# Anton-Le/PhysicsBasedBayesianInference

Measured on AMD Instinct MI355X. Metric: leapfrog-steps*chains/sec (node); d=128 Gaussian, ensemble=65536, higher is better.
Workload: dtype f64; 1 GPU; C2: d=128 dense-precision Gaussian, fp64, L=10 leapfrog steps per HMC iteration, in-kernel Philox momentum + Metropolis; chains_per_gpu=65536, total_chains=65536, D=128, L=10, parallelism=ensemble-sharded x1, draw=f32 (single-precision Box-Muller on the transcendental unit; momenta only)

## Files before the change

### physicsbasedbayesianinference_amd/csrc/kernels_dense.hip

```cpp
#include "kernels_dense_dev.h"

namespace {

struct DenseEvalPrm {
    const double* frag;
    const double* mu;
    const double* q;
    const double* p;
    const double* mass;
    double* U_out;
    double* grad_out;
    double* w_out;
    int64_t N, ldn;
    double cst;
    int D, mode;
};

template <int NT, bool FULL>
__global__ void __launch_bounds__(BLOCK, 1) k_dense_eval(DenseEvalPrm prm) {
    constexpr int DP = 16 * NT;
    constexpr int KS = 4 * NT;
    extern __shared__ __attribute__((aligned(16))) char smem[];
    v2f64* frag2 = reinterpret_cast<v2f64*>(smem);
    double* mu = reinterpret_cast<double*>(smem + (size_t)DP * DP * sizeof(double));
// ... 188 lines not shown
        return pbbi_fail(PBBI_ERR_UNSUPPORTED,
                         "dense kernels address a lane's rows with 32-bit offsets: padded D * "
                         "leading stride must be < 2^29 elements; shard the ensemble");
    return PBBI_OK;
}

int check(const pbbi_potential* pot) {
    if (pot->dtype != PBBI_F64)
        return pbbi_fail(PBBI_ERR_UNSUPPORTED, "dense Gaussian kernels are fp64 only in this build");
    if (pot->DP == 0 || pot->d_frag == nullptr)
        return pbbi_fail(PBBI_ERR_UNSUPPORTED,
                         "dense Gaussian: register-resident MFMA path needs D <= 128 (D = " +
                             std::to_string(pot->D) + ")");
    return PBBI_OK;
}

}

int dense_build_fragments(pbbi_potential* pot, const double* P, const double* mean) {
    const int D = pot->D;
    pot->DP = 0;
    pot->d_frag = nullptr;
    pot->d_mean_pad = nullptr;
    if (D > 128 || pot->dtype != PBBI_F64) return PBBI_OK;
    const int DP = D <= 32 ? 32 : (D <= 64 ? 64 : (D <= 96 ? 96 : 128));
    const int NT = DP / 16, KS = DP / 4;
    std::vector<double> frag((size_t)DP * DP, 0.0), mu((size_t)DP, 0.0);
    for (int s = 0; s < KS; ++s)
        for (int t = 0; t < NT; ++t)
            for (int l = 0; l < 64; ++l) {
                const int i = 16 * t + (l & 15), k = 4 * s + (l >> 4);
                const double val = (i < D && k < D) ? P[(size_t)i * D + k] : 0.0;
                frag[(((size_t)s * (NT / 2) + t / 2) * 64 + l) * 2 + (t & 1)] = val;
            }
    pot->zero_mean = true;
    for (int d = 0; d < D; ++d) {
        mu[d] = mean ? mean[d] : 0.0;
        if (mu[d] != 0.0) pot->zero_mean = false;
    }
    PBBI_HIP(hipMalloc(&pot->d_frag, frag.size() * sizeof(double)));
    PBBI_HIP(hipMalloc(&pot->d_mean_pad, mu.size() * sizeof(double)));
    PBBI_HIP(hipMemcpy(pot->d_frag, frag.data(), frag.size() * sizeof(double), hipMemcpyHostToDevice));
    PBBI_HIP(hipMemcpy(pot->d_mean_pad, mu.data(), mu.size() * sizeof(double), hipMemcpyHostToDevice));
    pot->DP = DP;
    return PBBI_OK;
}

int dense_hmc_iter(const IterArgs& a) {
    if (int rc = check(a.pot)) return rc;
    if (pbbi_dyn(a) && (a.method != PBBI_LEAPFROG || a.L < 1))
        return pbbi_fail(PBBI_ERR_UNSUPPORTED, "per-chain trajectory lengths on the dense kernel: Leapfrog with L >= 1");
    if (int rc = check_ld(a.pot, a.ldn_in > a.ldn_out ? a.ldn_in : a.ldn_out)) return rc;
    if (a.N == 0) return PBBI_OK;
    DensePrm prm{};
#ifdef PBBI_STAMPS
    prm.stamps = g_stamp_buf;
#endif
    prm.frag = (const double*)a.pot->d_frag;
    prm.mu = (const double*)a.pot->d_mean_pad;
    prm.q_in = (const double*)a.q_in;
    prm.p_in = (const double*)a.p_in;
    prm.u_in = (const double*)a.u_in;
    prm.mass = (const double*)a.mass;
    prm.q_out = (double*)a.q_out;
    prm.p_out = (double*)a.p_out;
    prm.v_out = nullptr;
    prm.ratio_out = (double*)a.ratio_out;
    prm.reject_out = a.reject_out;
    prm.N = a.N; prm.ldn_in = a.ldn_in; prm.ldn_out = a.ldn_out;
    prm.h = a.h; prm.cst = a.pot->cst; prm.kT = a.kT;
    prm.L = a.L; prm.D = a.pot->D; prm.flags = a.flags; prm.rng = a.rng; prm.mode = 0;
    prm.seed = a.seed; prm.iter = a.iter; prm.chain0 = a.chain0;
    prm.steps_in = a.steps_in; prm.steps_out = a.steps_out;
    int carry = 0;
    if (a.carry && a.carry_g && a.carry_sel && dense_carry_applies(a)) {
        carry = a.carry;
        prm.carry_g = (double*)a.carry_g;
        prm.carry_sel = a.carry_sel;
        prm.carry_slab_bytes = (uint32_t)((uint64_t)a.pot->DP * (uint64_t)a.N * 8u);
    }
    if (a.fuse_S > 1) {
        if (carry == 0 || a.ldn_in != a.ldn_out || !a.rng)
            return pbbi_fail(PBBI_ERR_INVALID, "fused dense iterations belong to a carried run (internal)");
        prm.fuse_first = (carry == 1);
        carry = 2;
        prm.fuse_S = a.fuse_S;
        prm.fuse_wrap2 = a.fuse_wrap2;
        prm.fuse_slab0 = a.fuse_slab0;
        prm.fuse_slab = (int64_t)a.pot->D * a.N;
        prm.fuse_q_base = (double*)a.fuse_q_base;
    } else if (carry != 0 && a.method == PBBI_STORMER_VERLET) {
        if (!a.rng) return pbbi_fail(PBBI_ERR_INVALID, "carried dense iterations draw in the kernel (internal)");
        prm.fuse_first = (carry == 1);
        carry = 2;
        prm.fuse_S = 1;
        prm.fuse_wrap2 = 0;
        prm.fuse_slab0 = 0;
        prm.fuse_slab = (int64_t)a.pot->D * a.N;
        prm.fuse_q_base = (double*)a.q_out;
    }
    return launch_traj(a.pot, a.method, prm, a.N, a.stream, carry);
}

int dense_fused_iterations(const IterArgs& a) {
    static const int chunk = [] {
        const char* e = getenv("PBBI_DENSE_FUSE");
// ... 66 lines not shown
```

### physicsbasedbayesianinference_amd/csrc/pbbi_api.hip

```cpp
#include <dlfcn.h>

#include <cmath>
#include <cstring>
#include <new>
#include <vector>

#include <type_traits>

#include "pbbi_internal.h"
#include "pbbi_chain.h"
#include "pbbi_rng.h"

static thread_local std::string g_last_error;

void pbbi_set_error(const std::string& msg) { g_last_error = msg; }
int pbbi_fail(int code, const std::string& msg) {
    g_last_error = msg;
    return code;
}

int pbbi_num_cus(int device) {
    static int cached[64] = {0};
    if (device >= 0 && device < 64 && cached[device]) return cached[device];
    int cus = 0;
// ... 584 lines not shown
int pbbi_device_count(int* count_out) {
    if (!count_out) return pbbi_fail(PBBI_ERR_INVALID, "count_out is NULL");
    *count_out = 0;
    PBBI_HIP(hipGetDeviceCount(count_out));
    return PBBI_OK;
}

int pbbi_device_info(int device, pbbi_devinfo* out) {
    if (!out) return pbbi_fail(PBBI_ERR_INVALID, "out is NULL");
    hipDeviceProp_t prop;
    PBBI_HIP(hipGetDeviceProperties(&prop, device));
    std::memset(out, 0, sizeof(*out));
    std::strncpy(out->name, prop.name, sizeof(out->name) - 1);
    std::strncpy(out->arch, prop.gcnArchName, sizeof(out->arch) - 1);
    out->compute_units = prop.multiProcessorCount;
    out->hbm_bytes = (int64_t)prop.totalGlobalMem;
    out->lds_bytes_per_block = (int)prop.sharedMemPerBlock;
    out->clock_khz = prop.clockRate;
    return PBBI_OK;
}

int pbbi_potential_create_harmonic(int D, const double* springConsts, int dtype, int device,
                                   pbbi_potential** out) {
    if (!springConsts) return pbbi_fail(PBBI_ERR_INVALID, "springConsts is NULL");
    if (int rc = new_handle(KIND_HARMONIC, D, dtype, device, out)) return rc;
    DeviceGuard guard(device);
    int rc = upload_padded(springConsts, D, dtype, &(*out)->d_prec);
    if (rc == PBBI_OK) rc = upload_mean(*out, nullptr);
    return finish_or_destroy(rc, out);
}

int pbbi_potential_create_gauss_diag(int D, const double* mean, const double* prec, double cst,
                                     int dtype, int device, pbbi_potential** out) {
    if (!prec) return pbbi_fail(PBBI_ERR_INVALID, "prec is NULL");
    if (int rc = new_handle(KIND_GAUSS_DIAG, D, dtype, device, out)) return rc;
    DeviceGuard guard(device);
    (*out)->cst = cst;
    int rc = upload_padded(prec, D, dtype, &(*out)->d_prec);
    if (rc == PBBI_OK) rc = upload_mean(*out, mean);
    return finish_or_destroy(rc, out);
}

int pbbi_potential_create_gauss_dense(int D, const double* mean, const double* precision,
                                      double cst, int dtype, int device, pbbi_potential** out) {
    if (!precision) return pbbi_fail(PBBI_ERR_INVALID, "precision is NULL");
    if (int rc = new_handle(KIND_GAUSS_DENSE, D, dtype, device, out)) return rc;
    DeviceGuard guard(device);
    (*out)->cst = cst;
    int rc = upload(precision, (size_t)D * D, dtype, &(*out)->d_prec);
    if (rc == PBBI_OK) rc = upload_mean(*out, mean);
    if (rc == PBBI_OK) rc = dense_build_fragments(*out, precision, mean);
    if (rc == PBBI_OK && (*out)->DP == 0) rc = big_build(*out, precision, mean);
    if (rc == PBBI_OK && (*out)->DP == 0) rc = dense_stream_build(*out, precision, mean);
    return finish_or_destroy(rc, out);
}

int pbbi_potential_create_rosenbrock(int D, double a, double b, double s, int dtype, int device,
                                     pbbi_potential** out) {
    if (!(s != 0.0)) return pbbi_fail(PBBI_ERR_INVALID, "Rosenbrock scale s must be non-zero");
    if (int rc = new_handle(KIND_ROSENBROCK, D, dtype, device, out)) return rc;
    (*out)->a = a; (*out)->b = b; (*out)->s = s;
    return PBBI_OK;
}

int pbbi_potential_create_custom(const char* plugin_path, int D, const double* params, int n_params,
                                 int dtype, int device, pbbi_potential** out) {
    if (!plugin_path) return pbbi_fail(PBBI_ERR_INVALID, "plugin_path is NULL");
    if (n_params < 0 || (n_params > 0 && !params))
        return pbbi_fail(PBBI_ERR_INVALID, "params is NULL / n_params < 0");
    if (int rc = new_handle(KIND_CUSTOM, D, dtype, device, out)) return rc;
    pbbi_potential* p = *out;
    DeviceGuard guard(device);
    p->plugin = dlopen(plugin_path, RTLD_NOW | RTLD_LOCAL);
    if (!p->plugin) {
        const char* why = dlerror();
        return finish_or_destroy(pbbi_fail(PBBI_ERR_INVALID, std::string("cannot load the potential plugin: ") +
                                                                 (why ? why : plugin_path)), out);
    }
    auto abi = (int (*)(void))dlsym(p->plugin, "pbbi_plugin_abi");
    auto pdt = (int (*)(void))dlsym(p->plugin, "pbbi_plugin_dtype");
    p->plugin_hmc_iter = (int (*)(const IterArgs*))dlsym(p->plugin, "pbbi_plugin_hmc_iter");
    p->plugin_integrate = (int (*)(const IntegrateArgs*))dlsym(p->plugin, "pbbi_plugin_integrate");
    p->plugin_eval = (int (*)(const EvalArgs*, int))dlsym(p->plugin, "pbbi_plugin_eval");
    int rc = PBBI_OK;
    if (!abi || !pdt || !p->plugin_hmc_iter || !p->plugin_integrate || !p->plugin_eval)
        rc = pbbi_fail(PBBI_ERR_INVALID, "plugin does not export the pbbi_plugin_* entry points");
    else if (abi() != PBBI_PLUGIN_ABI)
        rc = pbbi_fail(PBBI_ERR_INVALID, "plugin was built against another libpbbi (ABI " +
                                             std::to_string(abi()) + ", expected " +
                                             std::to_string(PBBI_PLUGIN_ABI) + "): rebuild it");
    else if (pdt() != dtype)
        rc = pbbi_fail(PBBI_ERR_INVALID, "plugin was built for the other dtype");
    if (rc == PBBI_OK) {
        p->n_params = n_params;
        rc = upload(params, (size_t)n_params, dtype, &p->d_params);
    }
    return finish_or_destroy(rc, out);
}

int pbbi_potential_create_glm(int D, int64_t M, const double* X, const double* y, int family,
                              double prior_precision, int dtype, int device, pbbi_potential** out) {
    if (!X || !y) return pbbi_fail(PBBI_ERR_INVALID, "X / y is NULL");
    if (M < 1) return pbbi_fail(PBBI_ERR_INVALID, "M must be >= 1");
    if (family != PBBI_GLM_LOGISTIC && family != PBBI_GLM_POISSON)
        return pbbi_fail(PBBI_ERR_INVALID, "unknown GLM family");
    if (!(prior_precision >= 0.0)) return pbbi_fail(PBBI_ERR_INVALID, "prior_precision must be >= 0");
    if (out) *out = nullptr;
    if (D > 128 || dtype == PBBI_F32)
        return pbbi_fail(PBBI_ERR_UNSUPPORTED, "GLM potentials run on the fp64 matrix-core kernels: float64 and "
                                               "D <= 128 only");
    if (int rc = new_handle(KIND_GLM, D, dtype, device, out)) return rc;
    DeviceGuard guard(device);
    return finish_or_destroy(glm_build(*out, M, X, y, family, prior_precision), out);
}

int pbbi_glm_pack_design(int D, int64_t M, const double* X, double* out, int64_t out_len, int64_t* len_out) {
    if (D < 1 || D > 128 || M < 1) return pbbi_fail(PBBI_ERR_INVALID, "need 1 <= D <= 128 and M >= 1");
    const int64_t len = glm_image_len(D, M);
    if (len_out) *len_out = len;
    if (!out) return PBBI_OK;
    if (!X) return pbbi_fail(PBBI_ERR_INVALID, "X is NULL");
    if (out_len < len) return pbbi_fail(PBBI_ERR_INVALID, "out is shorter than the image");
    glm_pack(D, M, X, out);
    return PBBI_OK;
}

int pbbi_potential_destroy(pbbi_potential* pot) {
    if (!pot) return PBBI_OK;
    DeviceGuard guard(pot->device);
    for (void* p : {pot->d_mean, pot->d_prec, pot->d_frag, pot->d_mean_pad, pot->d_big_PT, pot->d_big_mu,
                    pot->d_sfrag, pot->d_smean, pot->d_params, pot->d_glm_img, pot->d_glm_y})
        if (p) (void)hipFree(p);
    if (pot->plugin) (void)dlclose(pot->plugin);
    delete pot;
    return PBBI_OK;
}

int pbbi_potential_dim(const pbbi_potential* pot) { return pot ? pot->D : PBBI_ERR_INVALID; }
int pbbi_potential_dtype(const pbbi_potential* pot) { return pot ? pot->dtype : PBBI_ERR_INVALID; }
int pbbi_potential_device(const pbbi_potential* pot) { return pot ? pot->device : PBBI_ERR_INVALID; }

int pbbi_potential_eval(const pbbi_potential* pot, const void* q, int64_t N, int64_t ldn,
                        void* U_out, void* grad_out, void* stream) {
    if (int rc = check_common(pot, N, ldn)) return rc;
    if (!q && N > 0) return pbbi_fail(PBBI_ERR_INVALID, "q is NULL");
    DeviceGuard guard(pot->device);
    EvalArgs a{pot, q, nullptr, nullptr, N, ldn, U_out, grad_out, nullptr, 0, (hipStream_t)stream};
    return route_eval(a);
}

int pbbi_integrate(const pbbi_potential* pot, int method, void* q, void* p, const void* mass,
                   void* v_out, int64_t N, int64_t ldn, double h, int L, void* stream) {
    if (int rc = check_common(pot, N, ldn)) return rc;
    if (method != PBBI_LEAPFROG && method != PBBI_STORMER_VERLET)
        return pbbi_fail(PBBI_ERR_INVALID, "Invalid integration method selected.");
    if (L < 0) return pbbi_fail(PBBI_ERR_INVALID, "numSteps must be >= 0");
    if ((!q || !p) && N > 0) return pbbi_fail(PBBI_ERR_INVALID, "q / p is NULL");
    DeviceGuard guard(pot->device);
    IntegrateArgs a{pot, method, q, p, mass, v_out, N, ldn, h, L, (hipStream_t)stream};
    return route_integrate(a);
}

int pbbi_leapfrog(const pbbi_potential* pot, void* q, void* p, const void* mass, int64_t N,
                  int64_t ldn, double h, int L, void* stream) {
    return pbbi_integrate(pot, PBBI_LEAPFROG, q, p, mass, nullptr, N, ldn, h, L, stream);
}

int pbbi_stormer_verlet(const pbbi_potential* pot, void* q, void* p, const void* mass, int64_t N,
                        int64_t ldn, double h, int L, void* stream) {
    return pbbi_integrate(pot, PBBI_STORMER_VERLET, q, p, mass, nullptr, N, ldn, h, L, stream);
}

int pbbi_energy(const pbbi_potential* pot, const void* q, const void* p, const void* mass,
                int64_t N, int64_t ldn, void* H_out, void* weight_out, void* stream) {
    if (int rc = check_common(pot, N, ldn)) return rc;
    if ((!q || !p) && N > 0) return pbbi_fail(PBBI_ERR_INVALID, "q / p is NULL");
    DeviceGuard guard(pot->device);
    EvalArgs a{pot, q, p, mass, N, ldn, H_out, nullptr, weight_out, 0, (hipStream_t)stream};
    return route_energy(a);
}

int pbbi_weights_ratio(const pbbi_potential* pot, const void* newQ, const void* newP,
                       const void* oldQ, const void* oldP, const void* mass, int64_t N,
                       int64_t ldn, void* ratio_out, void* stream) {
    if (int rc = check_common(pot, N, ldn)) return rc;
    if (!ratio_out && N > 0) return pbbi_fail(PBBI_ERR_INVALID, "ratio_out is NULL");
// ... 241 lines not shown
    if (N == 0 || R < 2 || parity + 1 >= R) return PBBI_OK;
    if (!q || !betas) return pbbi_fail(PBBI_ERR_INVALID, "q / betas is NULL");
    DeviceGuard guard(pot->device);
    hipStream_t st = (hipStream_t)stream;
    Scratch ws(st);
    void* U = ws.get((size_t)N * elem_size(pot->dtype));
    if (!U) return pbbi_fail(PBBI_ERR_HIP, "hipMallocAsync failed for the potential energies");
    EvalArgs e{pot, q, nullptr, nullptr, N, ldn, U, nullptr, nullptr, 0, st};
    if (int rc = route_eval(e)) return rc;
    const int pairs = (R - parity) / 2;
    const dim3 grid((unsigned)((Nr + 255) / 256), (unsigned)pairs), block(256);
    if (pot->dtype == PBBI_F64)
        hipLaunchKernelGGL(k_replica_exchange<double>, grid, block, 0, st, (double*)q, ldn, (const double*)U, betas,
                           pot->D, Nr, R, parity, seed, iter, chain0, swapped_out);
    else
        hipLaunchKernelGGL(k_replica_exchange<float>, grid, block, 0, st, (float*)q, ldn, (const float*)U, betas,
                           pot->D, Nr, R, parity, seed, iter, chain0, swapped_out);
    PBBI_HIP(hipGetLastError());
    return PBBI_OK;
}

int pbbi_describe_run(const pbbi_potential* pot, int method, int64_t N, int64_t ldn, int L, int S, int flags,
                      char* out, int out_len) {
    if (int rc = hmc_check(pot, method, N, ldn, L)) return rc;
    if (!out || out_len < 1) return pbbi_fail(PBBI_ERR_INVALID, "out buffer missing");
    IterArgs a{};
    a.pot = pot; a.method = method; a.N = N; a.ldn_in = ldn; a.ldn_out = N; a.L = L; a.flags = flags; a.rng = 1;
    a.kT = 1.0;
    a.carry = 2; a.carry_g = (void*)(uintptr_t)16; a.carry_sel = (uint8_t*)(uintptr_t)16;
    std::string d;
    int fuse = 1;
    if (pot->kind == KIND_GLM) {
        d = "k_glm: GLM likelihood as two fp64 MFMA products per gradient (eta = X W, g = X^T r), 16 chains per wave, X "
            "staged through LDS in blocks of 16 observations (rows padded to " + std::to_string(pot->glm_DP) + ")";
        fuse = 1;
    } else if (pot->kind == KIND_CUSTOM) {
        d = "user-potential plugin kernels (one chain per lane; registers up to D = 16 / 32, workspace beyond)";
        fuse = route_fused_iterations(a);
    } else if (is_big(pot) && dense_stream_applies(a)) {
        d = "k_dense_hmc (streamed P): register-resident MFMA kernel, 16 chains per wave, one wave per SIMD, the "
            "precision matrix streamed through an LDS ring (rows padded to " + std::to_string(pot->DPS) + ")";
        const bool carry = S >= 2 && dense_stream_carry_applies(a);
        d += carry ? "; gradient carried between iterations: yes (L mat-vecs per iteration)"
                   : "; gradient carried between iterations: no (L + 1 mat-vecs per iteration)";
        if (!carry) a.carry = 0;
        fuse = carry ? dense_stream_fused_iterations(a) : 1;
    } else if (is_big(pot)) {
        d = "kernels_big: one fused MFMA GEMM per leapfrog step over the whole ensemble";
        d += big_carry_applies(a) && S >= 2 ? "; gradient carried between iterations: yes (L GEMMs per iteration)"
                                            : "; gradient carried between iterations: no (L + 1 GEMMs per iteration)";
    } else if (is_dense(pot)) {
        d = "k_dense_hmc: register-resident MFMA kernel, 16 chains per wave";
        const bool carry = S >= 2 && dense_carry_applies(a);
        if (carry) {
            d += "; gradient carried between iterations: yes (L mat-vecs per iteration)";
        } else {
            d += "; gradient carried between iterations: no (L + 1 mat-vecs per iteration) -- ";
            const uint64_t lim = (PBBI_CARRY_MAX_BYTES - 1) / ((uint64_t)pot->DP * 16u);
            if (S < 2) d += "a run of one iteration";
            else if (L < 1 || pbbi_dyn(a)) d += "runs of a fixed trajectory length L >= 1 only";
            else if ((uint64_t)N > lim)
                d += "the two carried-gradient slabs (D*N*16 bytes) must stay below 2^32 for 32-bit buffer offsets: "
                     "at D = " + std::to_string(pot->D) + " (rows padded to " + std::to_string(pot->DP) + ") that is N <= " + std::to_string(lim) +
                     " chains per call; shard the ensemble or split the call";
            else d += "switched off (PBBI_NO_CARRY / PBBI_DENSE_V1)";
        }
        if (!carry) a.carry = 0;
        fuse = carry ? dense_fused_iterations(a) : 1;
    } else {
        d = lane_route_name(a);
        fuse = lane_fused_iterations(a);
    }
    d += "; iterations per launch: up to " + std::to_string(fuse < 1 ? 1 : fuse);
    if (flags & PBBI_DRAW_F64) d += "; momentum draw: double precision";
    snprintf(out, (size_t)out_len, "%s", d.c_str());
    return PBBI_OK;
}

int pbbi_philox_normal(uint64_t seed, int rng_stream, uint64_t iter, uint64_t chain0, int D,
                       int64_t N, int64_t ldn, double scale, const void* scale_per_chain,
                       int dtype, int device, void* out, void* stream) {
    if (D < 1 || N < 0 || ldn < N) return pbbi_fail(PBBI_ERR_INVALID, "bad D / N / ldn");
    if (iter > UINT32_MAX) return pbbi_fail(PBBI_ERR_INVALID, "iter must be < 2^32");
    if (!out && N > 0) return pbbi_fail(PBBI_ERR_INVALID, "out is NULL");
    if (N == 0) return PBBI_OK;
    DeviceGuard guard(device);
    const dim3 grid((unsigned)((N + 255) / 256)), block(256);
    if (dtype == PBBI_F64)
        hipLaunchKernelGGL(k_philox_normal<double>, grid, block, 0, (hipStream_t)stream, seed,
                           rng_stream, iter, chain0, D, N, ldn, scale,
                           (const double*)scale_per_chain, (double*)out);
    else if (dtype == PBBI_F32)
        hipLaunchKernelGGL(k_philox_normal<float>, grid, block, 0, (hipStream_t)stream, seed,
                           rng_stream, iter, chain0, D, N, ldn, scale, (const float*)scale_per_chain,
                           (float*)out);
    else
        return pbbi_fail(PBBI_ERR_INVALID, "unknown dtype");
    PBBI_HIP(hipGetLastError());
    return PBBI_OK;
}

int pbbi_philox_steps(uint64_t seed, uint64_t iter, uint64_t chain0, int64_t N, int L, int device,
                      int32_t* out, void* stream) {
    if (N < 0 || L < 0) return pbbi_fail(PBBI_ERR_INVALID, "bad N / L");
    if (iter > UINT32_MAX) return pbbi_fail(PBBI_ERR_INVALID, "iter must be < 2^32");
    if (!out && N > 0) return pbbi_fail(PBBI_ERR_INVALID, "out is NULL");
    if (N == 0) return PBBI_OK;
// ... 174 lines not shown
```

### physicsbasedbayesianinference_amd/csrc/pbbi_internal.h

```cpp
#pragma once
#include <hip/hip_runtime.h>
#include <stdint.h>

#include <string>

#include "pbbi.h"

enum { KIND_HARMONIC = 0, KIND_GAUSS_DIAG = 1, KIND_GAUSS_DENSE = 2, KIND_ROSENBROCK = 3, KIND_CUSTOM = 4, KIND_GLM = 5 };

#define PBBI_PLUGIN_ABI 4

struct IterArgs;
struct IntegrateArgs;
struct EvalArgs;

struct pbbi_potential {
    int kind;
    int D;
    int dtype;
    int device;
    double cst, a, b, s;
    void* d_mean;
    void* d_prec;
    int DP;
    void* d_frag;
    void* d_mean_pad;
    bool zero_mean;
    int DPAD_big;
    void* d_big_PT;
    void* d_big_mu;
    void* plugin;
    void* d_params;
    int n_params;
    int (*plugin_hmc_iter)(const IterArgs*);
    int (*plugin_integrate)(const IntegrateArgs*);
    int (*plugin_eval)(const EvalArgs*, int mode);
    int DPS;
    void* d_sfrag;
    void* d_smean;
    int glm_DP;
    int glm_family;
    int64_t glm_M;
    double glm_lam;
    void* d_glm_img;
    void* d_glm_y;
};

void pbbi_set_error(const std::string& msg);
int pbbi_fail(int code, const std::string& msg);

#define PBBI_HIP(expr)                                                                          \
    do {                                                                                        \
        hipError_t _e = (expr);                                                                 \
        if (_e != hipSuccess)                                                                   \
            return pbbi_fail(PBBI_ERR_HIP, std::string(#expr) + ": " + hipGetErrorString(_e)); \
    } while (0)

struct DeviceGuard {
    int prev = -1;
    bool ok = true;
    explicit DeviceGuard(int dev) {
        if (hipGetDevice(&prev) != hipSuccess) { ok = false; return; }
        if (prev != dev && hipSetDevice(dev) != hipSuccess) ok = false;
    }
    ~DeviceGuard() {
        if (prev >= 0) (void)hipSetDevice(prev);
    }
};

__host__ __device__ inline double pbbi_accept_beta(int flags, double kT) {
    return (flags & PBBI_BETA_ACCEPT) ? 1.0 / kT : 1.0;
}

int pbbi_num_cus(int device);
struct IterArgs {
    const pbbi_potential* pot;
    int method;
    const void* q_in;
    const void* p_in;
    const void* u_in;
    const void* mass;
    void* q_out;
    void* p_out;
    void* ratio_out;
    uint8_t* reject_out;
    int64_t N, ldn_in, ldn_out;
    double h;
    int L;
    int flags;
    int rng;
    uint64_t seed, iter, chain0;
    double kT;
    hipStream_t stream;
    void* scratch;
    size_t scratch_bytes;
    size_t* scratch_used;
    int fuse_S;
    int fuse_wrap2;
// ... 56 lines not shown
        void* p = nullptr;
        if (hipMallocAsync(&p, bytes, st) != hipSuccess) return nullptr;
        owned.push_back(p);
        return p;
    }
    ~Scratch() {
        for (void* p : owned) (void)hipFreeAsync(p, st);
        if (used) *used = total;
    }
};

int lane_hmc_iter(const IterArgs& a);
int lane_integrate(const IntegrateArgs& a);
int lane_eval(const EvalArgs& a);
int lane_energy(const EvalArgs& a);
bool lane2_applies(const IterArgs& a);
int lane2_hmc_iter(const IterArgs& a);
int lane_fused_iterations(const IterArgs& a);
const char* lane_route_name(const IterArgs& a);
int lane_dyn_hmc_iter(const IterArgs& a);
bool lane_gist_applies(const pbbi_potential* pot);
int lane_gist_iter(const IterArgs& a);
bool sepn_applies(const IterArgs& a);
int sepn_hmc_iter(const IterArgs& a);
bool sepx_applies(const IterArgs& a);
int sepx_hmc_iter(const IterArgs& a);
bool rosn_applies(const IterArgs& a);
int rosn_hmc_iter(const IterArgs& a);
bool rosg_applies(const IterArgs& a);
int rosg_hmc_iter(const IterArgs& a);
bool rosgx_applies(const IterArgs& a);
int rosgx_hmc_iter(const IterArgs& a);
int stream_hmc_iter(const IterArgs& a);
int stream_integrate(const IntegrateArgs& a);
int stream_eval(const EvalArgs& a);
int stream_energy(const EvalArgs& a);
#define PBBI_CARRY_MAX_BYTES (((uint64_t)1 << 32) - ((uint64_t)1 << 20))
int dense_hmc_iter(const IterArgs& a);
bool dense_carry_applies(const IterArgs& a);
int dense_fused_iterations(const IterArgs& a);
bool big_carry_applies(const IterArgs& a);
void big_carry_bytes(const pbbi_potential* pot, int64_t N, size_t* g_bytes, size_t* sel_bytes);
int dense_integrate(const IntegrateArgs& a);
int dense_eval(const EvalArgs& a);
int dense_energy(const EvalArgs& a);
int dense_build_fragments(pbbi_potential* pot, const double* precision_host, const double* mean_host);
int dense_stream_build(pbbi_potential* pot, const double* precision_host, const double* mean_host);
bool dense_stream_applies(const IterArgs& a);
bool dense_stream_carry_applies(const IterArgs& a);
int dense_stream_fused_iterations(const IterArgs& a);
int dense_stream_hmc_iter(const IterArgs& a);
bool dense_stream_integrate_applies(const IntegrateArgs& a);
int dense_stream_integrate(const IntegrateArgs& a);
int big_hmc_iter(const IterArgs& a);
int big_integrate(const IntegrateArgs& a);
int big_eval(const EvalArgs& a);
int big_energy(const EvalArgs& a);
int big_build(pbbi_potential* pot, const double* precision_host, const double* mean_host);
int glm_build(pbbi_potential* pot, int64_t M, const double* X, const double* y, int family, double lam);
int glm_padded_dim(int D);
int64_t glm_image_len(int D, int64_t M);
void glm_pack(int D, int64_t M, const double* X, double* out);
int glm_hmc_iter(const IterArgs& a);
int glm_integrate(const IntegrateArgs& a);
int glm_eval(const EvalArgs& a);
int glm_energy(const EvalArgs& a);
```

Before: 2.086 billion leapfrog-steps*chains/s.

## Apply L leapfrog steps as one precomputed linear propagator for dense Gaussians

For a D=128 fp64 dense Gaussian, leapfrog dynamics are linear, so the L steps collapse into one map. The map's blocks are built from a host-side Jacobi eigendecomposition of the precision matrix and baked into device images, cached per (h, L). A new MFMA kernel then does a fixed five mat-vecs per HMC iteration instead of L, streaming the images through an LDS ring with buffer-to-LDS loads. The cost is setup work, extra device memory for the images and eigenvectors, and rounding that can differ from stepwise integration. The path runs only when L is at least 7 and no per-chain mass is given.

```diff
diff --git a/physicsbasedbayesianinference_amd/csrc/kernels_dense.hip b/physicsbasedbayesianinference_amd/csrc/kernels_dense.hip
--- a/physicsbasedbayesianinference_amd/csrc/kernels_dense.hip
+++ b/physicsbasedbayesianinference_amd/csrc/kernels_dense.hip
@@ -264,6 +264,7 @@
         return pbbi_fail(PBBI_ERR_UNSUPPORTED, "per-chain trajectory lengths on the dense kernel: Leapfrog with L >= 1");
     if (int rc = check_ld(a.pot, a.ldn_in > a.ldn_out ? a.ldn_in : a.ldn_out)) return rc;
     if (a.N == 0) return PBBI_OK;
+    if (a.carry && a.carry_g && a.carry_sel && dense_prop_applies(a)) return dense_prop_hmc_iter(a);
     DensePrm prm{};
 #ifdef PBBI_STAMPS
     prm.stamps = g_stamp_buf;
diff --git a/physicsbasedbayesianinference_amd/csrc/kernels_dprop.hip b/physicsbasedbayesianinference_amd/csrc/kernels_dprop.hip
--- /dev/null
+++ b/physicsbasedbayesianinference_amd/csrc/kernels_dprop.hip
@@ -0,0 +1,557 @@
+#include <cmath>
+#include <mutex>
+
+#include "kernels_dense_dev.h"
+
+namespace {
+
+constexpr int PROP_MIN_L_DEFAULT = 7;
+
+struct PropCfg {
+    static constexpr int CHUNK = 16384;
+    static constexpr int RING = 4;
+    static constexpr int DMA = 4;
+    static constexpr int NCYC = 40;
+    static constexpr int C_A1 = 0, C_G = 8, C_B = 16, C_A2 = 24, C_P = 32;
+    static constexpr int LDS_RING = RING * CHUNK;
+    static constexpr int LDS = LDS_RING + 128 * 8;
+    static constexpr size_t IMG_DOUBLES = (size_t)NCYC * CHUNK / 8;
+};
+
+__device__ __forceinline__ void pr_issue_part(const PRing& r, int ci, int m) {
+    using C = PropCfg;
+    typedef __attribute__((address_space(3))) void lds_void;
+    const int slot = ci % C::RING;
+    __builtin_amdgcn_raw_ptr_buffer_load_lds(r.src, (lds_void*)(r.lds + slot * C::CHUNK + m * 4096), 16, r.voff,
+                                             (uint32_t)(ci * C::CHUNK + m * 4096) + r.woff, 0, 0);
+}
+
+template <int KC, bool INLOOP>
+__device__ __forceinline__ void pr_acquire() {
+    using C = PropCfg;
+    constexpr int YOUNGER = INLOOP ? C::DMA * (C::RING - 3) + (C::DMA < KC - 1 ? C::DMA : KC - 1) : C::DMA * (C::RING - 2);
+    asm volatile("s_waitcnt vmcnt(%0) lgkmcnt(0)\n\ts_barrier" ::"n"(YOUNGER) : "memory");
+}
+
+template <int HP, int C0, bool ZERO, typename XF, typename PF>
+__device__ __forceinline__ void prop_pass(const PRing& r, const v2f64* __restrict__ ringL, v4f64 (&acc)[2 * HP], XF xat,
+                                          PF pre) {
+    using C = PropCfg;
+    constexpr int KS = 32, KC = 16 / HP, H1 = (HP + 1) / 2;
+    auto frag_at = [&](int s, int t2) -> v2f64 {
+        const int slot = (C0 + s / KC) % C::RING;
+        return ringL[((slot * KC + s % KC) * HP + t2) * 64];
+    };
+    pr_acquire<KC, false>();
+    v2f64 A[HP], An[HP];
+#pragma unroll
+    for (int t2 = 0; t2 < HP; ++t2) A[t2] = frag_at(0, t2);
+    if constexpr (ZERO) {
+#pragma unroll
+        for (int t = 0; t < 2 * HP; ++t) acc[t] = v4f64{0.0, 0.0, 0.0, 0.0};
+    }
+    double x = xat(0);
+#pragma unroll
+    for (int s = 0; s < KS; ++s) {
+#pragma unroll
+        for (int t2 = 0; t2 < H1; ++t2) {
+            acc[2 * t2] = __builtin_amdgcn_mfma_f64_16x16x4f64(A[t2].x, x, acc[2 * t2], 0, 0, 0);
+            acc[2 * t2 + 1] = __builtin_amdgcn_mfma_f64_16x16x4f64(A[t2].y, x, acc[2 * t2 + 1], 0, 0, 0);
+        }
+        __builtin_amdgcn_sched_barrier(0);
+        if (s + 1 < KS) {
+            if ((s + 1) % KC == 0) pr_acquire<KC, true>();
+#pragma unroll
+            for (int t2 = 0; t2 < HP; ++t2) An[t2] = frag_at(s + 1, t2);
+            pre(s + 1);
+        }
+        __builtin_amdgcn_sched_barrier(0);
+#pragma unroll
+        for (int t2 = H1; t2 < HP; ++t2) {
+            acc[2 * t2] = __builtin_amdgcn_mfma_f64_16x16x4f64(A[t2].x, x, acc[2 * t2], 0, 0, 0);
+            acc[2 * t2 + 1] = __builtin_amdgcn_mfma_f64_16x16x4f64(A[t2].y, x, acc[2 * t2 + 1], 0, 0, 0);
+        }
+        __builtin_amdgcn_sched_barrier(0);
+        if (s % KC < C::DMA) pr_issue_part(r, (C0 + s / KC + C::RING - 1) % C::NCYC, s % KC);
+        if (s + 1 < KS) x = xat(s + 1);
+#pragma unroll
+        for (int t2 = 0; t2 < HP; ++t2) A[t2] = An[t2];
+    }
+}
+
+__device__ __forceinline__ double dot16(const double* x, const v4f64 (&acc)[4]) {
+    double sum = 0.0;
+#pragma unroll
+    for (int t = 0; t < 4; ++t)
+#pragma unroll
+        for (int r = 0; r < 4; ++r) sum = fma(x[4 * t + r], acc[t][r], sum);
+    return sum;
+}
+
+template <bool ZMEAN, int DRAW>
+__global__ void __launch_bounds__(BLOCK, 2) k_dense_hmc_prop(DensePrm prm) {
+    using C = PropCfg;
+    constexpr int KS = 32;
+    extern __shared__ __attribute__((aligned(16))) char smem[];
+    const int lane = threadIdx.x & 63;
+    const int wave = __builtin_amdgcn_readfirstlane(threadIdx.x >> 6);
+    double* mu = reinterpret_cast<double*>(smem + C::LDS_RING);
+    PRing ring{};
+    ring.src = buf_make(prm.frag);
+    ring.lds = smem + wave * 1024;
+    ring.voff = 16u * (uint32_t)lane;
+    ring.woff = 1024u * (uint32_t)wave;
+    if (prm.fuse_first) {
+#pragma unroll
+        for (int ci = 0; ci < C::RING - 1; ++ci)
+#pragma unroll
+            for (int m = 0; m < C::DMA; ++m) pr_issue_part(ring, C::C_P + ci, m);
+    } else {
+#pragma unroll
+        for (int ci = 0; ci < C::RING - 1; ++ci)
+#pragma unroll
+            for (int m = 0; m < C::DMA; ++m) pr_issue_part(ring, ci, m);
+    }
+    for (int i = threadIdx.x; i < 128; i += BLOCK) mu[i] = prm.mu[i];
+    __syncthreads();
+    if (blockIdx.x & 1) __builtin_amdgcn_s_setprio(1);
+    const int g = lane >> 4;
+    const int c = lane & 15;
+    const v2f64* ringL = reinterpret_cast<const v2f64*>(smem) + lane;
+    const double* muG = mu + g;
+
+    int64_t n0 = ((int64_t)blockIdx.x * 4 + wave) * CHAINS_PER_WAVE;
+    bool ghost = false;
+    if (n0 >= prm.N) {
+        ghost = true;
+        n0 = (prm.N - 1) / CHAINS_PER_WAVE * CHAINS_PER_WAVE;
+    }
+    const int64_t left = prm.N - n0;
+    const bool valid = !ghost && c < left;
+    const int cc = c < left ? c : (int)left - 1;
+    const uint32_t ld_in = 8u * (uint32_t)prm.ldn_in, ld_out = 8u * (uint32_t)prm.ldn_out;
+    const uint32_t vin = (uint32_t)g * ld_in + 8u * (uint32_t)cc, s4in = 4u * ld_in;
+    const uint32_t vout = (uint32_t)g * ld_out + 8u * (uint32_t)cc, s4out = 4u * ld_out;
+    const __amdgpu_buffer_rsrc_t qin = buf_make(prm.q_in + n0);
+    const uint32_t ld_g = 8u * (uint32_t)prm.N, s4g = 4u * ld_g;
+    const uint32_t vg0 = (uint32_t)g * ld_g + 8u * (uint32_t)cc;
+    const __amdgpu_buffer_rsrc_t gbuf = buf_make(prm.carry_g + n0);
+    uint32_t csel = prm.fuse_first ? 0u : prm.carry_sel[n0 + cc];
+    const uint64_t chain = prm.chain0 + (uint64_t)(n0 + cc);
+    const double pstd = sqrt(prm.kT);
+    auto nopre = [](int) {};
+    using I0 = std::integral_constant<int, 0>;
+    using I1 = std::integral_constant<int, 1>;
+
+    double xL[KS];
+    v4f64 acc[8];
+    double xg_cur = 0.0;
+    auto grad_pass = [&](auto pass_c, uint32_t voff) -> double {
+        constexpr int PASS = decltype(pass_c)::value;
+        v4f64 (&a4)[4] = reinterpret_cast<v4f64 (&)[4]>(acc[0]);
+        prop_pass<2, C::C_P + 4 * PASS, true>(ring, ringL, a4, [&](int s) { return xL[s]; }, nopre);
+        if (valid) {
+#pragma unroll
+            for (int t = 0; t < 4; ++t)
+#pragma unroll
+                for (int r = 0; r < 4; ++r) store_row(gbuf, voff, s4g, 4 * (PASS * 4 + t) + r, a4[t][r]);
+        }
+        return dot16(xL + 16 * PASS, a4);
+    };
+    if (prm.fuse_first) {
+#pragma unroll
+        for (int s = 0; s < KS; ++s) {
+            const double qv = load_row(qin, vin, s4in, s);
+            xL[s] = ZMEAN ? qv : qv - muG[4 * s];
+        }
+        xg_cur = grad_pass(I0{}, vg0);
+        xg_cur += grad_pass(I1{}, vg0);
+    } else {
+        const uint32_t vgc = vg0 + (csel ? prm.carry_slab_bytes : 0u);
+        double part[2];
+#pragma unroll
+        for (int pass = 0; pass < 2; ++pass) {
+            double sum = 0.0;
+#pragma unroll
+            for (int i = 0; i < 16; ++i) {
+                const int s = 16 * pass + i;
+                const double qv = load_row(qin, vin, s4in, s);
+                sum = fma(ZMEAN ? qv : qv - muG[4 * s], load_row(gbuf, vgc, s4g, s), sum);
+            }
+            part[pass] = sum;
+        }
+        xg_cur = part[0] + part[1];
+    }
+    __builtin_amdgcn_sched_barrier(0);
+
+#pragma nounroll
+    for (int kf = 0; kf < prm.fuse_S; ++kf) {
+        const uint64_t iter_k = prm.iter + (uint64_t)kf;
+        double* const ratio_k = prm.ratio_out ? prm.ratio_out + (int64_t)kf * prm.N : nullptr;
+        uint8_t* const reject_k = prm.reject_out ? prm.reject_out + (int64_t)kf * prm.N : nullptr;
+        const int64_t s_out = prm.fuse_wrap2 ? ((prm.fuse_slab0 + kf) & 1) : prm.fuse_slab0 + kf;
+        const int64_t s_prev = prm.fuse_wrap2 ? ((prm.fuse_slab0 + kf - 1) & 1) : prm.fuse_slab0 + kf - 1;
+        const __amdgpu_buffer_rsrc_t qin_k = kf > 0 ? buf_make(prm.fuse_q_base + s_prev * prm.fuse_slab + n0) : qin;
+        const uint32_t vq = kf > 0 ? vout : vin, s4q = kf > 0 ? s4out : s4in;
+        const __amdgpu_buffer_rsrc_t qout_k = buf_make(prm.fuse_q_base + s_out * prm.fuse_slab + n0);
+        const __amdgpu_buffer_rsrc_t pout_k = buf_make(prm.p_out + (prm.p_out ? (int64_t)kf * prm.fuse_slab : 0) + n0);
+        const bool have_p = (prm.p_out != nullptr);
+        const uint32_t vg_cur = vg0 + (csel ? prm.carry_slab_bytes : 0u);
+        const uint32_t vg_new = vg0 + (csel ? 0u : prm.carry_slab_bytes);
+
+        double xa[8], xb[8];
+        auto g0_load = [&](double (&dst)[8], int grp) {
+#pragma unroll
+            for (int i = 0; i < 8; ++i) dst[i] = load_row(gbuf, vg_cur, s4g, 8 * grp + i);
+        };
+        auto x0_load = [&](double (&dst)[8], int grp) {
+#pragma unroll
+            for (int i = 0; i < 8; ++i) {
+                const double qv = load_row(qin_k, vq, s4q, 8 * grp + i);
+                dst[i] = qv;
+            }
+        };
+        g0_load(xa, 0);
+
+        double p[KS];
+        const bool draw64 = DRAW == 1;
+#pragma unroll
+        for (int k = 0; k < KS / 4; ++k) {
+            double z[4];
+            rng_normal4d(prm.seed, PBBI_STREAM_MOMENTUM, iter_k, chain, (uint32_t)((k << 2) | g), draw64, z);
+#pragma unroll
+            for (int sl = 0; sl < 4; ++sl) p[4 * k + sl] = z[sl] * pstd;
+            __builtin_amdgcn_sched_barrier(0);
+        }
+        double pp = 0.0;
+#pragma unroll
+        for (int s = 0; s < KS; ++s) pp += p[s] * p[s];
+        const double oldH = 0.5 * chain_sum(pp) + (0.5 * chain_sum(xg_cur) + prm.cst);
+
+        prop_pass<4, C::C_A1, true>(ring, ringL, acc, [&](int s) { return p[s]; }, nopre);
+        prop_pass<4, C::C_G, false>(
+            ring, ringL, acc, [&](int s) { return ((s >> 3) & 1) ? xb[s & 7] : xa[s & 7]; },
+            [&](int s) {
+                if (s % 8 == 1 && s / 8 + 1 < 4) {
+                    if ((s / 8 + 1) & 1) g0_load(xb, s / 8 + 1);
+                    else g0_load(xa, s / 8 + 1);
+                }
+            });
+        __builtin_amdgcn_sched_barrier(0);
+        x0_load(xa, 0);
+        pp = 0.0;
+#pragma unroll
+        for (int t = 0; t < 8; ++t)
+#pragma unroll
+            for (int r = 0; r < 4; ++r) pp += acc[t][r] * acc[t][r];
+        if (have_p && valid) {
+#pragma unroll
+            for (int t = 0; t < 8; ++t)
+#pragma unroll
+                for (int r = 0; r < 4; ++r) store_row(pout_k, vout, s4out, 4 * t + r, acc[t][r]);
+        }
+        __builtin_amdgcn_sched_barrier(0);
+
+        prop_pass<4, C::C_B, true>(ring, ringL, acc, [&](int s) { return p[s]; }, nopre);
+        prop_pass<4, C::C_A2, false>(
+            ring, ringL, acc,
+            [&](int s) {
+                const double qv = ((s >> 3) & 1) ? xb[s & 7] : xa[s & 7];
+                return ZMEAN ? qv : qv - muG[4 * s];
+            },
+            [&](int s) {
+                if (s % 8 == 1 && s / 8 + 1 < 4) {
+                    if ((s / 8 + 1) & 1) x0_load(xb, s / 8 + 1);
+                    else x0_load(xa, s / 8 + 1);
+                }
+            });
+        __builtin_amdgcn_sched_barrier(0);
+#pragma unroll
+        for (int t = 0; t < 8; ++t)
+#pragma unroll
+            for (int r = 0; r < 4; ++r) {
+                const int s = 4 * t + r;
+                const double qv = ZMEAN ? acc[t][r] : acc[t][r] + muG[4 * s];
+                if (valid) store_row(qout_k, vout, s4out, s, qv);
+                xL[s] = ZMEAN ? qv : qv - muG[4 * s];
+            }
+        __builtin_amdgcn_sched_barrier(0);
+
+        double xg_new = grad_pass(I0{}, vg_new);
+        xg_new += grad_pass(I1{}, vg_new);
+
+        const double newH = 0.5 * chain_sum(pp) + (0.5 * chain_sum(xg_new) + prm.cst);
+        const double ratio = exp((oldH - newH) * pbbi_accept_beta(prm.flags, prm.kT));
+        const double u = rng_uniform(prm.seed, iter_k, chain);
+        const bool reject = (ratio == ratio) && (u > (ratio < 1.0 ? ratio : 1.0));
+        if (reject) {
+            const bool compat = (prm.flags & PBBI_COMPAT_P_FROM_OLDQ) != 0;
+#pragma unroll
+            for (int s = 0; s < KS; ++s) xL[s] = load_row(qin_k, vq, s4q, s);
+            if (valid) {
+#pragma unroll
+                for (int s = 0; s < KS; ++s) store_row(qout_k, vout, s4out, s, xL[s]);
+                if (have_p) {
+#pragma unroll
+                    for (int s = 0; s < KS; ++s) store_row(pout_k, vout, s4out, s, compat ? xL[s] : p[s]);
+                }
+            }
+        }
+        csel ^= reject ? 0u : 1u;
+        xg_cur = reject ? xg_cur : xg_new;
+        if (valid && g == 0) {
+            if (ratio_k) ratio_k[n0 + c] = ratio;
+            if (reject_k) reject_k[n0 + c] = reject ? 1 : 0;
+        }
+    }
+    if (valid && g == 0) prm.carry_sel[n0 + c] = (uint8_t)csel;
+    asm volatile("s_waitcnt vmcnt(0)" ::: "memory");
+}
+
+__host__ __device__ inline double prop_vfv(const double* __restrict__ V, const double* __restrict__ f, int i, int k) {
+    double s = 0.0, e = 0.0;
+    for (int m = 0; m < 128; ++m) {
+        const double a = V[i * 128 + m], b = V[k * 128 + m], w = f[m];
+        const double ab = a * b, abe = fma(a, b, -ab);
+        const double t = ab * w, te = fma(ab, w, -t);
+        const double sn = s + t, bb = sn - s;
+        e += ((s - (sn - bb)) + (t - bb)) + (te + abe * w);
+        s = sn;
+    }
+    return s + e;
+}
+
+__global__ void k_prop_images(const double* __restrict__ V, const double* __restrict__ coef ,
+                              const double* __restrict__ P, double* __restrict__ out) {
+    const int idx = blockIdx.x * blockDim.x + threadIdx.x;
+    if (idx >= (int)PropCfg::IMG_DOUBLES) return;
+    const int img = idx / 16384, w = idx % 16384;
+    const int e = w & 1, l = (w >> 1) & 63;
+    int i, k;
+    if (img < 4) {
+        const int t2 = (w >> 7) & 3, s = w >> 9;
+        i = 16 * (2 * t2 + e) + (l & 15);
+        k = 4 * s + (l >> 4);
+    } else {
+        const int t2 = (w >> 7) & 1, s = (w >> 8) & 31, pass = w >> 13;
+        i = 16 * (pass * 4 + 2 * t2 + e) + (l & 15);
+        k = 4 * s + (l >> 4);
+    }
+    const int sel = img == 0 ? 0 : img == 1 ? 1 : img == 2 ? 2 : 0;
+    out[idx] = img == 4 ? P[i * 128 + k] : prop_vfv(V, coef + 128 * sel, i, k);
+}
+
+void jacobi_eig(int n, std::vector<long double>& a, std::vector<long double>& v, std::vector<long double>& w) {
+    v.assign((size_t)n * n, 0.0L);
+    for (int i = 0; i < n; ++i) v[(size_t)i * n + i] = 1.0L;
+    long double norm = 0.0L;
+    for (long double x : a) norm += x * x;
+    for (int sweep = 0; sweep < 60; ++sweep) {
+        long double off = 0.0L;
+        for (int p = 0; p < n; ++p)
+            for (int q = p + 1; q < n; ++q) off += a[(size_t)p * n + q] * a[(size_t)p * n + q];
+        if (off <= 1e-42L * norm) break;
+        for (int p = 0; p < n; ++p)
+            for (int q = p + 1; q < n; ++q) {
+                const long double apq = a[(size_t)p * n + q];
+                if (apq == 0.0L) continue;
+                const long double theta = (a[(size_t)q * n + q] - a[(size_t)p * n + p]) / (2.0L * apq);
+                const long double t = (theta >= 0 ? 1.0L : -1.0L) / (fabsl(theta) + sqrtl(theta * theta + 1.0L));
+                const long double cs = 1.0L / sqrtl(t * t + 1.0L), sn = t * cs;
+                for (int k = 0; k < n; ++k) {
+                    const long double akp = a[(size_t)k * n + p], akq = a[(size_t)k * n + q];
+                    a[(size_t)k * n + p] = cs * akp - sn * akq;
+                    a[(size_t)k * n + q] = sn * akp + cs * akq;
+                }
+                for (int k = 0; k < n; ++k) {
+                    const long double apk = a[(size_t)p * n + k], aqk = a[(size_t)q * n + k];
+                    a[(size_t)p * n + k] = cs * apk - sn * aqk;
+                    a[(size_t)q * n + k] = sn * apk + cs * aqk;
+                }
+                for (int k = 0; k < n; ++k) {
+                    const long double vkp = v[(size_t)k * n + p], vkq = v[(size_t)k * n + q];
+                    v[(size_t)k * n + p] = cs * vkp - sn * vkq;
+                    v[(size_t)k * n + q] = sn * vkp + cs * vkq;
+                }
+            }
+    }
+    w.resize(n);
+    for (int i = 0; i < n; ++i) w[i] = a[(size_t)i * n + i];
+}
+
+void prop_coefficients(const std::vector<long double>& lam, double h, int L, double* a_out, double* g_out, double* b_out) {
+    const long double hl = (long double)h;
+    for (size_t i = 0; i < lam.size(); ++i) {
+        long double a = 1.0L, b = 0.0L, cg = 0.0L, d = 1.0L;
+        const long double l = lam[i];
+        for (int j = 0; j < L; ++j) {
+            cg -= 0.5L * hl * a;  d -= 0.5L * hl * l * b;
+            a += hl * l * cg;     b += hl * d;
+            cg -= 0.5L * hl * a;  d -= 0.5L * hl * l * b;
+        }
+        a_out[i] = (double)(0.5L * (a + d));
+        g_out[i] = (double)cg;
+        b_out[i] = (double)b;
+    }
+}
+
+struct PropCache {
+    std::mutex mtx;
+    std::vector<double> P;
+    std::vector<long double> lam;
+    std::vector<double> V;
+    double* d_V = nullptr;
+    double* d_coef = nullptr;
+    double* d_img = nullptr;
+    double h = 0.0;
+    int L = -1;
+};
+
+void prop_factor(PropCache* pc) {
+    if (!pc->V.empty()) return;
+    std::vector<long double> a(pc->P.begin(), pc->P.end()), v;
+    for (int i = 0; i < 128; ++i)
+        for (int k = i + 1; k < 128; ++k) a[i * 128 + k] = a[k * 128 + i] = 0.5L * (a[i * 128 + k] + a[k * 128 + i]);
+    jacobi_eig(128, a, v, pc->lam);
+    pc->V.assign(v.begin(), v.end());
+}
+
+int prop_images(const pbbi_potential* pot, double h, int L, hipStream_t st, const double** out) {
+    PropCache* pc = (PropCache*)pot->prop;
+    std::lock_guard<std::mutex> lock(pc->mtx);
+    if (pc->d_img && pc->h == h && pc->L == L) {
+        *out = pc->d_img;
+        return PBBI_OK;
+    }
+    prop_factor(pc);
+    if (!pc->d_V) {
+        double* dv = nullptr;
+        PBBI_HIP(hipMalloc((void**)&dv, 128 * 128 * sizeof(double)));
+        if (hipMemcpy(dv, pc->V.data(), 128 * 128 * sizeof(double), hipMemcpyHostToDevice) != hipSuccess) {
+            (void)hipFree(dv);
+            return pbbi_fail(PBBI_ERR_HIP, "propagator set-up: upload of the eigenvectors failed");
+        }
+        pc->d_V = dv;
+    }
+    if (!pc->d_coef) PBBI_HIP(hipMalloc((void**)&pc->d_coef, 3 * 128 * sizeof(double)));
+    if (pc->d_img) (void)hipFree(pc->d_img);
+    pc->d_img = nullptr;
+    pc->L = -1;
+    double coef[3 * 128];
+    prop_coefficients(pc->lam, h, L, coef, coef + 128, coef + 256);
+    PBBI_HIP(hipMemcpy(pc->d_coef, coef, sizeof(coef), hipMemcpyHostToDevice));
+    PBBI_HIP(hipMalloc((void**)&pc->d_img, PropCfg::IMG_DOUBLES * sizeof(double)));
+    hipLaunchKernelGGL(k_prop_images, dim3((unsigned)(PropCfg::IMG_DOUBLES / 256)), dim3(256), 0, st, pc->d_V, pc->d_coef,
+                       (const double*)pot->d_prec, pc->d_img);
+    PBBI_HIP(hipGetLastError());
+    pc->h = h;
+    pc->L = L;
+    *out = pc->d_img;
+    return PBBI_OK;
+}
+
+}
+
+int dense_prop_build(pbbi_potential* pot, const double* P) {
+    pot->prop = nullptr;
+    if (pot->D != 128 || pot->dtype != PBBI_F64) return PBBI_OK;
+    PropCache* pc = new (std::nothrow) PropCache();
+    if (!pc) return pbbi_fail(PBBI_ERR_INVALID, "out of host memory");
+    pc->P.assign(P, P + 128 * 128);
+    pot->prop = pc;
+    return PBBI_OK;
+}
+
+void dense_prop_destroy(pbbi_potential* pot) {
+    PropCache* pc = (PropCache*)pot->prop;
+    if (!pc) return;
+    for (void* p : {(void*)pc->d_V, (void*)pc->d_coef, (void*)pc->d_img})
+        if (p) (void)hipFree(p);
+    delete pc;
+    pot->prop = nullptr;
+}
+
+bool dense_prop_applies(const IterArgs& a) {
+    static const bool off = (getenv("PBBI_NO_PROPAGATOR") != nullptr);
+    static const int min_l = [] {
+        const char* e = getenv("PBBI_PROP_MIN_L");
+        const int v = e ? atoi(e) : PROP_MIN_L_DEFAULT;
+        return v < 1 ? 1 : v;
+    }();
+    const pbbi_potential* pot = a.pot;
+    return !off && pot->kind == KIND_GAUSS_DENSE && pot->prop != nullptr && pot->DP == 128 && pot->D == 128 &&
+           a.method == PBBI_LEAPFROG && a.mass == nullptr && a.rng && a.L >= min_l && dense_carry_applies(a);
+}
+
+int dense_prop_hmc_iter(const IterArgs& a) {
+    const pbbi_potential* pot = a.pot;
+    if (!dense_prop_applies(a) || !a.carry || !a.carry_g || !a.carry_sel)
+        return pbbi_fail(PBBI_ERR_INVALID, "dense propagator kernel: not applicable (internal)");
+    if ((int64_t)pot->DP * (a.ldn_in > a.ldn_out ? a.ldn_in : a.ldn_out) >= ((int64_t)1 << 29))
+        return pbbi_fail(PBBI_ERR_UNSUPPORTED, "dense kernels address a lane's rows with 32-bit offsets: padded D * "
+                                               "leading stride must be < 2^29 elements; shard the ensemble");
+    if (a.N == 0) return PBBI_OK;
+    const double* img = nullptr;
+    if (int rc = prop_images(pot, a.h, a.L, a.stream, &img)) return rc;
+    DensePrm prm{};
+    prm.frag = img;
+    prm.mu = (const double*)pot->d_mean_pad;
+    prm.q_in = (const double*)a.q_in;
+    prm.q_out = (double*)a.q_out;
+    prm.p_out = (double*)a.p_out;
+    prm.ratio_out = (double*)a.ratio_out;
+    prm.reject_out = a.reject_out;
+    prm.N = a.N; prm.ldn_in = a.ldn_in; prm.ldn_out = a.ldn_out;
+    prm.h = a.h; prm.cst = pot->cst; prm.kT = a.kT;
+    prm.L = a.L; prm.D = pot->D; prm.flags = a.flags; prm.rng = 1; prm.mode = 0;
+    prm.seed = a.seed; prm.iter = a.iter; prm.chain0 = a.chain0;
+    prm.carry_g = (double*)a.carry_g;
+    prm.carry_sel = a.carry_sel;
+    prm.carry_slab_bytes = (uint32_t)((uint64_t)pot->DP * (uint64_t)a.N * 8u);
+    prm.fuse_first = (a.carry == 1);
+    prm.fuse_slab = (int64_t)pot->D * a.N;
+    if (a.fuse_S > 1) {
+        prm.fuse_S = a.fuse_S;
+        prm.fuse_wrap2 = a.fuse_wrap2;
+        prm.fuse_slab0 = a.fuse_slab0;
+        prm.fuse_q_base = (double*)a.fuse_q_base;
+    } else {
+        prm.fuse_S = 1;
+        prm.fuse_wrap2 = 0;
+        prm.fuse_slab0 = 0;
+        prm.fuse_q_base = (double*)a.q_out;
+    }
+    const dim3 grid((unsigned)((a.N + CHAINS_PER_WG - 1) / CHAINS_PER_WG)), block(BLOCK);
+    const size_t lds = PropCfg::LDS;
+#define LAUNCH_P(Z_, DR_)                                                                                  \
+    {                                                                                                      \
+        auto k = k_dense_hmc_prop<Z_, DR_>;                                                                \
+        PBBI_HIP(hipFuncSetAttribute(reinterpret_cast<const void*>(k), hipFuncAttributeMaxDynamicSharedMemorySize, \
+                                     (int)lds));                                                           \
+        hipLaunchKernelGGL(k, grid, block, lds, a.stream, prm);                                            \
+    }
+    const bool d64 = (a.flags & PBBI_DRAW_F64) != 0;
+    if (pot->zero_mean) {
+        if (d64) LAUNCH_P(true, 1) else LAUNCH_P(true, 0)
+    } else {
+        if (d64) LAUNCH_P(false, 1) else LAUNCH_P(false, 0)
+    }
+#undef LAUNCH_P
+    PBBI_HIP(hipGetLastError());
+    return PBBI_OK;
+}
+
+extern "C" int pbbi_debug_propagator_images(int D, const double* P, double h, int L, double* coef_out, double* A_out,
+                                            double* G_out, double* B_out) {
+    if (D != 128 || !P || L < 1 || !coef_out || !A_out || !G_out || !B_out)
+        return pbbi_fail(PBBI_ERR_INVALID, "propagator images: D = 128, L >= 1, non-NULL outputs");
+    PropCache pc;
+    pc.P.assign(P, P + 128 * 128);
+    prop_factor(&pc);
+    prop_coefficients(pc.lam, h, L, coef_out, coef_out + 128, coef_out + 256);
+    double* outs[3] = {A_out, G_out, B_out};
+    for (int im = 0; im < 3; ++im)
+        for (int i = 0; i < 128; ++i)
+            for (int k = 0; k < 128; ++k) outs[im][i * 128 + k] = prop_vfv(pc.V.data(), coef_out + 128 * im, i, k);
+    return PBBI_OK;
+}
diff --git a/physicsbasedbayesianinference_amd/csrc/pbbi_api.hip b/physicsbasedbayesianinference_amd/csrc/pbbi_api.hip
--- a/physicsbasedbayesianinference_amd/csrc/pbbi_api.hip
+++ b/physicsbasedbayesianinference_amd/csrc/pbbi_api.hip
@@ -660,6 +660,7 @@
     if (rc == PBBI_OK) rc = dense_build_fragments(*out, precision, mean);
     if (rc == PBBI_OK && (*out)->DP == 0) rc = big_build(*out, precision, mean);
     if (rc == PBBI_OK && (*out)->DP == 0) rc = dense_stream_build(*out, precision, mean);
+    if (rc == PBBI_OK && (*out)->DP == 128) rc = dense_prop_build(*out, precision);
     return finish_or_destroy(rc, out);
 }
 
@@ -740,6 +741,7 @@
                     pot->d_sfrag, pot->d_smean, pot->d_params, pot->d_glm_img, pot->d_glm_y})
         if (p) (void)hipFree(p);
     if (pot->plugin) (void)dlclose(pot->plugin);
+    dense_prop_destroy(pot);
     delete pot;
     return PBBI_OK;
 }
@@ -1087,7 +1089,12 @@
     } else if (is_dense(pot)) {
         d = "k_dense_hmc: register-resident MFMA kernel, 16 chains per wave";
         const bool carry = S >= 2 && dense_carry_applies(a);
-        if (carry) {
+        if (carry && dense_prop_applies(a)) {
+            d = "k_dense_hmc (L-step propagator): register-resident MFMA kernel, 16 chains per wave, the L leapfrog steps "
+                "applied as one linear map whose images stream through an LDS ring; gradient carried between iterations: yes "
+                "(5 mat-vecs per iteration whatever L is, L-step propagator; a run with per-chain masses takes the stepwise "
+                "kernel)";
+        } else if (carry) {
             d += "; gradient carried between iterations: yes (L mat-vecs per iteration)";
         } else {
             d += "; gradient carried between iterations: no (L + 1 mat-vecs per iteration) -- ";
diff --git a/physicsbasedbayesianinference_amd/csrc/pbbi_internal.h b/physicsbasedbayesianinference_amd/csrc/pbbi_internal.h
--- a/physicsbasedbayesianinference_amd/csrc/pbbi_internal.h
+++ b/physicsbasedbayesianinference_amd/csrc/pbbi_internal.h
@@ -44,6 +44,7 @@
     double glm_lam;
     void* d_glm_img;
     void* d_glm_y;
+    void* prop;
 };
 
 void pbbi_set_error(const std::string& msg);
@@ -206,6 +207,10 @@
 int dense_stream_hmc_iter(const IterArgs& a);
 bool dense_stream_integrate_applies(const IntegrateArgs& a);
 int dense_stream_integrate(const IntegrateArgs& a);
+int dense_prop_build(pbbi_potential* pot, const double* precision_host);
+void dense_prop_destroy(pbbi_potential* pot);
+bool dense_prop_applies(const IterArgs& a);
+int dense_prop_hmc_iter(const IterArgs& a);
 int big_hmc_iter(const IterArgs& a);
 int big_integrate(const IntegrateArgs& a);
 int big_eval(const EvalArgs& a);
```

Result: faster. 3.558 billion leapfrog-steps*chains/s, median of 6 (+70.6%).
